# IlzeAmandaA/VAE-GP-ODE

Measured on AMD Instinct MI355X. Metric: latent_trajectories_per_sec, higher is better.
Workload: dtype f32; 1 GPU; configs[1]: ode1 DF q=6 M=100 S=256 T=16 batch=256; step = full ELBO training step (encoder, GP draw, rk4 rollout, decoder, ELBO, backward, Adam), L=1; global_batch=256, mc_draws=1, solver=rk4 (3/8 rule), parallelism=dp1, hip_graph=True, graph_scope=whole, gp_side_stream=True, batchnorm=per-process statistics

## Files before the change

vae-gp-ode_amd/csrc/conv_fwd_v2.hpp:

```cpp
#pragma once
#include "conv_mfma.hpp"

namespace gp {

template <class L> struct FwV2 {
  using PL = FwdPolicy<L, L::CO>;
  template <int CLS> using C = typename PL::template C<CLS>;
  static constexpr int KC = L::CI, NC = L::CO, KK = L::K * L::K, KG = KC / 4;
  static_assert(NC == 16 && L::S == 2 && PL::NCLS == 4, "one co tile, four stride-parity classes");
  static constexpr int NKS = KK * KG;
  static constexpr int NPX = C<0>::npc;
  static_assert(C<1>::npc == NPX && C<2>::npc == NPX && C<3>::npc == NPX && C<1>::nx == C<0>::nx && C<2>::nx == C<0>::nx &&
                C<3>::nx == C<0>::nx, "the classes share one q-grid");
  static constexpr int SH = L::HI, OHW = L::HO * L::HO;
  static constexpr int SRC = KC * SH * SH;
  static constexpr int PS = PL::PS, HP = PL::HP, PADL = PL::PADL, IMG = KC * PS;
  static constexpr int NCW = 4, NTHR = 64 * (NCW + 4), NLT = NTHR - 64 * NCW;
  static constexpr int TPW = 2;
  static constexpr int WIN = 16 * NCW * TPW;
  static constexpr int PF = 2;
  static constexpr int NBUF = (2 * WIN - 2) / NPX + 2;
  static constexpr int MAXS = PADL * (HP + 1);
  static constexpr int TFO = (HP * HP + 3) / 4 * 4;
  static_assert(igemm_tf_in_pad<PL>(), "the input-transform table fits the plane tails");
  static_assert(TPW * (PF + 1) <= 15, "LDS reads in flight within what lgkmcnt counts");
  static_assert(NPX <= 256 && SRC % 4 == 0 && SH * SH <= NLT, "float4 source, producer offset table");
  static_assert(4 * (MAXS + (KG - 1) * 4 * PS) < 65536, "operand offsets fit the ds_read immediate");
  static constexpr int CST = NBUF * IMG;
  static constexpr int IPG = 2, NSW = 8;
  static constexpr int RED = CST + 2 * NC;
  static constexpr size_t lds_bytes(bool stats) { return sizeof(float) * ((size_t)RED + (stats ? (NSW + 1) * 2 * NC : 0)); }
};

template <class E, int PY>
__device__ __forceinline__ void fwv2_pair(const float* __restrict__ s_buf, const int (&base)[2][E::TPW], const float (&wr)[E::NKS],
                                          f32x4 (&acc)[2][E::TPW]) {
  using G0 = typename E::template C<2 * PY>;
  using G1 = typename E::template C<2 * PY + 1>;
  constexpr int N0 = G0::ntaps * E::KG, N = N0 + G1::ntaps * E::KG, W0 = G0::slab_taps * E::KG;
  static_assert(G1::slab_taps == G0::slab_taps + G0::ntaps, "class-major weight registers");
  float bf[E::PF + 1][E::TPW];
  auto fetch = [&](auto sc) {
    constexpr int S = decltype(sc)::value, c = S >= N0 ? 1 : 0, s = c ? S - N0 : S;
    const int off = E::MAXS + (c ? G1::tap_off(s / E::KG) : G0::tap_off(s / E::KG)) + (s % E::KG) * 4 * E::PS;
#pragma unroll
    for (int t = 0; t < E::TPW; ++t) bf[S % (E::PF + 1)][t] = s_buf[base[c][t] + off];
  };
#pragma unroll
  for (int t = 0; t < E::TPW; ++t) acc[0][t] = acc[1][t] = f32x4{0.f, 0.f, 0.f, 0.f};
  static_for<E::PF>([&](auto sc) { fetch(sc); });
  static_for<N>([&](auto sc) {
    constexpr int S = decltype(sc)::value, c = S >= N0 ? 1 : 0;
    if constexpr (S + E::PF < N) fetch(std::integral_constant<int, S + E::PF>{});
    __builtin_amdgcn_sched_barrier(0);
#pragma unroll
    for (int t = 0; t < E::TPW; ++t) acc[c][t] = __builtin_amdgcn_mfma_f32_16x16x4f32(wr[W0 + S], bf[S % (E::PF + 1)][t], acc[c][t], 0, 0, 0);
    __builtin_amdgcn_sched_barrier(0);
  });
}

template <class L, bool HAS_BN, bool STATS>
__global__ __launch_bounds__(FwV2<L>::NTHR) void k_conv_fwd_v2(const float* __restrict__ x, const float* __restrict__ w,
                                                               const float* __restrict__ bias, float* __restrict__ y, int B,
                                                               const float* __restrict__ in_bn, BnSink sink) {
  using E = FwV2<L>;
  constexpr int KC = E::KC, NC = E::NC, KK = E::KK, KG = E::KG, NPX = E::NPX, IMG = E::IMG, PS = E::PS, HP = E::HP, WIN = E::WIN;
  constexpr int SH = E::SH, PADL = E::PADL, NLT = E::NLT, NBUF = E::NBUF, TPW = E::TPW, NCW = E::NCW, OHW = E::OHW;
  float* s_buf = igemm_smem;
  const int tid = threadIdx.x, lane = tid & 63, wave = __builtin_amdgcn_readfirstlane(tid >> 6);
  const int bx = blockIdx.x, ngx = gridDim.x, ngroups = (B + E::IPG - 1) / E::IPG;
  const int ngrp = bx < ngroups ? (ngroups - 1 - bx) / ngx + 1 : 0;
  const int nit = STATS ? (ngrp ? E::IPG * (ngrp - 1) + min(E::IPG, B - E::IPG * (bx + (ngrp - 1) * ngx)) : 0)
                        : (bx < B ? (B - 1 - bx) / ngx + 1 : 0);
  auto img = [&](int j) { return STATS ? E::IPG * (bx + (j / E::IPG) * ngx) + j % E::IPG : bx + j * ngx; };
  const int npx = nit * NPX, nwin = (npx + WIN - 1) / WIN;
  auto last_img = [&](int i) { return min(nit - 1, (i * WIN + WIN - 1) / NPX); };

  for (int e = tid; e < NBUF * IMG / 4; e += E::NTHR) reinterpret_cast<float4*>(s_buf)[e] = float4{0.f, 0.f, 0.f, 0.f};
  if (tid < NC) {
    s_buf[E::CST + tid] = bias ? bias[tid] : 0.f;
    s_buf[E::CST + NC + tid] = STATS ? bn_sink_shift(sink, tid) : 0.f;
  }
  __syncthreads();
  if constexpr (HAS_BN) {
    for (int e = tid; e < KC; e += E::NTHR) *reinterpret_cast<float4*>(s_buf + e * PS + E::TFO) = reinterpret_cast<const float4*>(in_bn)[e];
    __syncthreads();
  }
  float bs[2][4] = {{0.f, 0.f, 0.f, 0.f}, {0.f, 0.f, 0.f, 0.f}}, bq[2][4] = {{0.f, 0.f, 0.f, 0.f}, {0.f, 0.f, 0.f, 0.f}};

  if (wave >= NCW) {
    __builtin_amdgcn_s_setprio(3);
    const int lt = tid - 64 * NCW;
    constexpr int N4 = E::SRC / 4;
    int otab[4], opl[4];
#pragma unroll
    for (int k = 0; k < 4; ++k) {
      const int e = 4 * min(lt, SH * SH - 1) + k, pl = e / (SH * SH), q = e % (SH * SH);
      opl[k] = pl * PS;
      otab[k] = pl * PS + (q / SH + PADL) * HP + q % SH + PADL;
    }
    auto stage = [&](int j) __attribute__((always_inline)) {
      const float4* src = reinterpret_cast<const float4*>(x) + (size_t)img(j) * N4;
      float* buf = s_buf + (j % NBUF) * IMG;
      if (lt < SH * SH) {
        float4 v[KG];
#pragma unroll
        for (int g = 0; g < KG; ++g) v[g] = src[g * SH * SH + lt];
#pragma unroll
        for (int g = 0; g < KG; ++g) {
          float* d = buf + 4 * g * PS;
          float e[4] = {v[g].x, v[g].y, v[g].z, v[g].w};
          if constexpr (HAS_BN) {
#pragma unroll
            for (int k = 0; k < 4; ++k) e[k] = bn_relu(e[k], *reinterpret_cast<const float4*>(s_buf + 4 * g * PS + opl[k] + E::TFO));
          }
          d[otab[0]] = e[0]; d[otab[1]] = e[1]; d[otab[2]] = e[2]; d[otab[3]] = e[3];
        }
      }
    };
    const int pw = wave - NCW, slr = lane & 15, slk = lane >> 4;
    float kk[4];
#pragma unroll
    for (int r = 0; r < 4; ++r) kk[r] = STATS ? s_buf[E::CST + NC + 4 * slk + r] : 0.f;
    auto stats_group = [&](int k) __attribute__((always_inline)) {
      const int b0 = E::IPG * (bx + k * ngx), mtot = min(E::IPG, B - b0) * NPX, njobs = (mtot + 15) / 16;
      constexpr int NT0 = E::template C<0>::ntaps + E::template C<1>::ntaps, NT1 = E::template C<2>::ntaps + E::template C<3>::ntaps;
      const int wtot = njobs * (NT0 + NT1);
#pragma unroll
      for (int e = 0; e < 2; ++e) {
        const int jw = 2 * pw + e, lo = (wtot * jw) / E::NSW, hi = (wtot * (jw + 1)) / E::NSW;
        static_for<2>([&](auto pyc) {
          constexpr int PY = decltype(pyc)::value, ntaps = PY ? NT1 : NT0;
          using G1 = typename E::template C<2 * PY + 1>;
          const int cbase = PY ? njobs * NT0 : 0;
          const int nlo = lo - cbase - ntaps / 2, nhi = hi - cbase - ntaps / 2;
          const int ub = min(njobs, nlo <= 0 ? 0 : (nlo + ntaps - 1) / ntaps), ue = min(njobs, nhi <= 0 ? 0 : (nhi + ntaps - 1) / ntaps);
          constexpr int U = 8;
          for (int u0 = ub; u0 < ue; u0 += U) {
            float2 v[U][4];
#pragma unroll
            for (int t = 0; t < U; ++t) {
              const int m = min((u0 + t) * 16 + slr, mtot - 1), im = m / NPX, p = m - im * NPX;
              const float* yp = y + ((size_t)(b0 + im) * NC + 4 * slk) * OHW + G1::out_off(p);
#pragma unroll
              for (int r = 0; r < 4; ++r) v[t][r] = *reinterpret_cast<const float2*>(yp + (size_t)r * OHW);
            }
#pragma unroll
            for (int t = 0; t < U; ++t) {
              if (u0 + t < ue && (u0 + t) * 16 + slr < mtot) {
#pragma unroll
                for (int r = 0; r < 4; ++r) {
                  const float d1 = v[t][r].x - kk[r], d0 = v[t][r].y - kk[r];
                  bs[e][r] += d1; bq[e][r] = fmaf(d1, d1, bq[e][r]);
                  bs[e][r] += d0; bq[e][r] = fmaf(d0, d0, bq[e][r]);
                }
              }
            }
          }
        });
      }
    };
    int staged = -1, summed = 0;
    if (nit > 0)
      for (; staged < last_img(0); ) stage(++staged);
    __syncthreads();
    for (int i = 0; i < nwin; ++i) {
      if (i + 1 < nwin)
        for (const int j1 = last_img(i + 1); staged < j1; ) stage(++staged);
      if constexpr (STATS) {
        __builtin_amdgcn_s_setprio(0);
        for (; summed < ngrp && min(npx, E::IPG * NPX * (summed + 1)) <= i * WIN; ++summed) stats_group(summed);
        __builtin_amdgcn_s_setprio(3);
      }
      __syncthreads();
    }
    __builtin_amdgcn_s_setprio(0);
    if constexpr (STATS)
      for (; summed < ngrp; ++summed) stats_group(summed);
  } else {
    const int lr = lane & 15, lk = lane >> 4;
    float wr[E::NKS];
    static_for<4>([&](auto cc) {
      using G = typename E::template C<decltype(cc)::value>;
#pragma unroll
      for (int s = 0; s < G::ntaps * KG; ++s) {
        const int t = s / KG, ky = G::py + L::S * (t / G::ntx), kx = G::px + L::S * (t % G::ntx);
        wr[G::slab_taps * KG + s] = w[((size_t)(4 * (s % KG) + lk) * NC + lr) * KK + ky * L::K + kx];
      }
    });
    __syncthreads();
    for (int i = 0; i < nwin; ++i) {
      const int t0 = i * WIN + 16 * wave;
      if (t0 < npx) {
        int jp[TPW];
#pragma unroll
        for (int t = 0; t < TPW; ++t) {
          const int m = min(t0 + 16 * NCW * t + lr, npx - 1);
          const int j = m / NPX;
          jp[t] = j << 8 | (m - j * NPX);
        }
        static_for<2>([&](auto pyc) {
          constexpr int PY = decltype(pyc)::value;
          using G0 = typename E::template C<2 * PY>;
          using G1 = typename E::template C<2 * PY + 1>;
          static_assert(G0::out_off(0) == G1::out_off(0) + 1 && G0::out_off(NPX - 1) == G1::out_off(NPX - 1) + 1 &&
                        G1::out_off(0) % 2 == 0 && L::HO % 2 == 0, "paired classes write neighbouring, 8-byte aligned columns");
          int base[2][TPW];
#pragma unroll
          for (int t = 0; t < TPW; ++t) {
            const int lb = ((jp[t] >> 8) % NBUF) * IMG + lk * PS - E::MAXS;
            base[0][t] = lb + G0::pix_addr(jp[t] & 255);
            base[1][t] = lb + G1::pix_addr(jp[t] & 255);
          }
          f32x4 acc[2][TPW];
          fwv2_pair<E, PY>(s_buf, base, wr, acc);
          const float4 b4 = *reinterpret_cast<const float4*>(s_buf + E::CST + 4 * lk);
          const float bv[4] = {b4.x, b4.y, b4.z, b4.w};
#pragma unroll
          for (int t = 0; t < TPW; ++t) {
            int c = jp[t];
            asm volatile("" : "+v"(c));
            if (t0 + 16 * NCW * t + lr < npx) {
              const int j = c >> 8;
              float* yp = y + ((size_t)img(j) * NC + 4 * lk) * OHW + G1::out_off(c & 255);
#pragma unroll
              for (int r = 0; r < 4; ++r) {
                const float v0 = acc[0][t][r] + bv[r], v1 = acc[1][t][r] + bv[r];
                *reinterpret_cast<float2*>(yp + (size_t)r * OHW) = float2{v1, v0};
              }
            }
          }
        });
      }
      __syncthreads();
    }
  }

  if constexpr (STATS) {
    float* red = s_buf + E::RED;
    float* s_sm = red + E::NSW * 2 * NC;
    const int lr = lane & 15, lk = lane >> 4;
#pragma unroll
    for (int e = 0; e < 2; ++e)
#pragma unroll
      for (int r = 0; r < 4; ++r) {
        const float a = row_allreduce16(bs[e][r]), b = row_allreduce16(bq[e][r]);
        if (lr == 0 && wave >= NCW) {
          red[((wave - NCW + NCW * e) * NC + 4 * lk + r) * 2] = a;
          red[((wave - NCW + NCW * e) * NC + 4 * lk + r) * 2 + 1] = b;
        }
      }
    __syncthreads();
    if (tid < 2 * NC) {
      float t = 0.f;
      for (int wv = 0; wv < E::NSW; ++wv) t += red[wv * 2 * NC + tid];
      s_sm[tid] = t;
    }
    __syncthreads();
    bn_sink_publish<NC, E::NTHR>(sink, s_sm);
  }
}

}
```

Baseline: 105,500 trajectories/s.

## Interleave BN stats chunks with input staging in conv forward loader waves

Replaces the per-group batch-norm statistics loop in the loader waves with a resumable segment iterator that processes one 8-job chunk per window. Each chunk's global loads are issued before the staging of the next window's inputs, and the sum is done afterward, so the stats load latency overlaps with staging instead of stalling whole groups at once. The two row-parity classes are merged through a constant output offset. This adds iterator bookkeeping and predicated register selects, and it spreads the stats work across windows, with the leftover chunks handled after the loop.

```diff
diff --git a/vae-gp-ode_amd/csrc/conv_fwd_v2.hpp b/vae-gp-ode_amd/csrc/conv_fwd_v2.hpp
--- a/vae-gp-ode_amd/csrc/conv_fwd_v2.hpp
+++ b/vae-gp-ode_amd/csrc/conv_fwd_v2.hpp
@@ -122,61 +122,97 @@
     float kk[4];
 #pragma unroll
     for (int r = 0; r < 4; ++r) kk[r] = STATS ? s_buf[E::CST + NC + 4 * slk + r] : 0.f;
-    auto stats_group = [&](int k) __attribute__((always_inline)) {
-      const int b0 = E::IPG * (bx + k * ngx), mtot = min(E::IPG, B - b0) * NPX, njobs = (mtot + 15) / 16;
-      constexpr int NT0 = E::template C<0>::ntaps + E::template C<1>::ntaps, NT1 = E::template C<2>::ntaps + E::template C<3>::ntaps;
-      const int wtot = njobs * (NT0 + NT1);
-#pragma unroll
-      for (int e = 0; e < 2; ++e) {
-        const int jw = 2 * pw + e, lo = (wtot * jw) / E::NSW, hi = (wtot * (jw + 1)) / E::NSW;
-        static_for<2>([&](auto pyc) {
-          constexpr int PY = decltype(pyc)::value, ntaps = PY ? NT1 : NT0;
-          using G1 = typename E::template C<2 * PY + 1>;
-          const int cbase = PY ? njobs * NT0 : 0;
-          const int nlo = lo - cbase - ntaps / 2, nhi = hi - cbase - ntaps / 2;
-          const int ub = min(njobs, nlo <= 0 ? 0 : (nlo + ntaps - 1) / ntaps), ue = min(njobs, nhi <= 0 ? 0 : (nhi + ntaps - 1) / ntaps);
-          constexpr int U = 8;
-          for (int u0 = ub; u0 < ue; u0 += U) {
-            float2 v[U][4];
-#pragma unroll
-            for (int t = 0; t < U; ++t) {
-              const int m = min((u0 + t) * 16 + slr, mtot - 1), im = m / NPX, p = m - im * NPX;
-              const float* yp = y + ((size_t)(b0 + im) * NC + 4 * slk) * OHW + G1::out_off(p);
-#pragma unroll
-              for (int r = 0; r < 4; ++r) v[t][r] = *reinterpret_cast<const float2*>(yp + (size_t)r * OHW);
-            }
-#pragma unroll
-            for (int t = 0; t < U; ++t) {
-              if (u0 + t < ue && (u0 + t) * 16 + slr < mtot) {
-#pragma unroll
-                for (int r = 0; r < 4; ++r) {
-                  const float d1 = v[t][r].x - kk[r], d0 = v[t][r].y - kk[r];
-                  bs[e][r] += d1; bq[e][r] = fmaf(d1, d1, bq[e][r]);
-                  bs[e][r] += d0; bq[e][r] = fmaf(d0, d0, bq[e][r]);
-                }
-              }
-            }
+    constexpr int U = 8;
+    constexpr int NT0 = E::template C<0>::ntaps + E::template C<1>::ntaps, NT1 = E::template C<2>::ntaps + E::template C<3>::ntaps;
+    constexpr int DPY = E::template C<3>::out_off(0) - E::template C<1>::out_off(0);
+    static_assert(E::template C<3>::out_off(NPX - 1) - E::template C<1>::out_off(NPX - 1) == DPY, "row parities differ by a constant offset");
+    int qk = 0, qs = 0, qu = -1;
+    int q_ue = 0, q_mtot = 0;
+    auto seg_next = [&]() __attribute__((always_inline)) {
+      while (qk < ngrp) {
+        const int b0 = E::IPG * (bx + qk * ngx), njobs = (min(E::IPG, B - b0) * NPX + 15) / 16;
+        const int wtot = njobs * (NT0 + NT1), jw = 2 * pw + (qs >> 1), lo = (wtot * jw) / E::NSW, hi = (wtot * (jw + 1)) / E::NSW;
+        q_mtot = min(E::IPG, B - b0) * NPX;
+        int ub;
+        if (qs & 1) {
+          const int nlo = lo - njobs * NT0 - NT1 / 2, nhi = hi - njobs * NT0 - NT1 / 2;
+          ub = min(njobs, nlo <= 0 ? 0 : (nlo + NT1 - 1) / NT1); q_ue = min(njobs, nhi <= 0 ? 0 : (nhi + NT1 - 1) / NT1);
+        } else {
+          const int nlo = lo - NT0 / 2, nhi = hi - NT0 / 2;
+          ub = min(njobs, nlo <= 0 ? 0 : (nlo + NT0 - 1) / NT0); q_ue = min(njobs, nhi <= 0 ? 0 : (nhi + NT0 - 1) / NT0);
+        }
+        if (qu < 0) qu = ub;
+        if (qu < q_ue) return true;
+        qu = -1;
+        if (++qs == 4) { qs = 0; ++qk; }
+      }
+      return false;
+    };
+    auto seg_end = [&]() { return E::IPG * NPX * qk + min(16 * min(qu + U, q_ue), q_mtot); };
+    auto seg_load = [&](float2 (&v)[U][4]) __attribute__((always_inline)) {
+      const float* yg = y + ((size_t)E::IPG * (bx + qk * ngx) * NC + 4 * slk) * OHW + ((qs & 1) ? DPY : 0);
+#pragma unroll
+      for (int t = 0; t < U; ++t) {
+        const int m = min((qu + t) * 16 + slr, q_mtot - 1), im = m / NPX, p = m - im * NPX;
+        const float* yp = yg + (size_t)im * NC * OHW + E::template C<1>::out_off(p);
+#pragma unroll
+        for (int r = 0; r < 4; ++r) v[t][r] = *reinterpret_cast<const float2*>(yp + (size_t)r * OHW);
+      }
+    };
+    auto seg_sum = [&](const float2 (&v)[U][4]) __attribute__((always_inline)) {
+      const bool e = qs >> 1;
+      float s[4], q[4];
+#pragma unroll
+      for (int r = 0; r < 4; ++r) { s[r] = e ? bs[1][r] : bs[0][r]; q[r] = e ? bq[1][r] : bq[0][r]; }
+#pragma unroll
+      for (int t = 0; t < U; ++t) {
+        if (qu + t < q_ue && (qu + t) * 16 + slr < q_mtot) {
+#pragma unroll
+          for (int r = 0; r < 4; ++r) {
+            const float d1 = v[t][r].x - kk[r], d0 = v[t][r].y - kk[r];
+            s[r] += d1; q[r] = fmaf(d1, d1, q[r]);
+            s[r] += d0; q[r] = fmaf(d0, d0, q[r]);
           }
-        });
-      }
-    };
-    int staged = -1, summed = 0;
+        }
+      }
+#pragma unroll
+      for (int r = 0; r < 4; ++r) {
+        bs[0][r] = e ? bs[0][r] : s[r]; bq[0][r] = e ? bq[0][r] : q[r];
+        bs[1][r] = e ? s[r] : bs[1][r]; bq[1][r] = e ? q[r] : bq[1][r];
+      }
+      qu += U;
+    };
+    int staged = -1;
     if (nit > 0)
       for (; staged < last_img(0); ) stage(++staged);
     __syncthreads();
-    for (int i = 0; i < nwin; ++i) {
+    auto stage_for = [&](int i) __attribute__((always_inline)) {
       if (i + 1 < nwin)
         for (const int j1 = last_img(i + 1); staged < j1; ) stage(++staged);
-      if constexpr (STATS) {
+    };
+    for (int i = 0; i < nwin; ++i) {
+      if (STATS && seg_next() && seg_end() <= i * WIN) {
+        float2 v[U][4];
         __builtin_amdgcn_s_setprio(0);
-        for (; summed < ngrp && min(npx, E::IPG * NPX * (summed + 1)) <= i * WIN; ++summed) stats_group(summed);
+        seg_load(v);
         __builtin_amdgcn_s_setprio(3);
+        stage_for(i);
+        __builtin_amdgcn_s_setprio(0);
+        seg_sum(v);
+        __builtin_amdgcn_s_setprio(3);
+      } else {
+        stage_for(i);
       }
       __syncthreads();
     }
     __builtin_amdgcn_s_setprio(0);
-    if constexpr (STATS)
-      for (; summed < ngrp; ++summed) stats_group(summed);
+    if constexpr (STATS) {
+      while (seg_next()) {
+        float2 v[U][4];
+        seg_load(v);
+        seg_sum(v);
+      }
+    }
   } else {
     const int lr = lane & 15, lk = lane >> 4;
     float wr[E::NKS];
```

After: 104,700 trajectories/s. Within noise of the previous version (-0.8%).
